# hassony2/homan

Hardware: AMD Instinct MI355X
Metric: optimisation iters/sec (30-frame 256^2 clip) (higher is better)
Workload: dtype f32

## Files before the change

### homan_amd/csrc/geometry.hip

```cpp
#include "hm_common.h"

__global__ __launch_bounds__(256) void k_rigid_fwd(const float* __restrict__ mesh, const float* __restrict__ rot6d,
                                                   const float* __restrict__ trans, const float* __restrict__ scale,
                                                   int abs_scale, int N, int V, float* __restrict__ rotmat,
                                                   float* __restrict__ verts, int clip_len)
{
    __shared__ float R[9];
    const int n = blockIdx.y;
    if (threadIdx.x == 0) {
        float r[9];
        rot6d_to_mat(rot6d + n * 6, r);
#pragma unroll
        for (int k = 0; k < 9; ++k) R[k] = r[k];
        if (blockIdx.x == 0 && rotmat)
#pragma unroll
            for (int k = 0; k < 9; ++k) rotmat[n * 9 + k] = r[k];
    }
    __syncthreads();
    const int v = blockIdx.x * blockDim.x + threadIdx.x;
    if (v >= V) return;
    float s = scale[n / clip_len];
    if (abs_scale) s = fabsf(s);
    const float* m = mesh + ((long)n * V + v) * 3;
    const float x = s * m[0], y = s * m[1], z = s * m[2];
    float* o = verts + ((long)n * V + v) * 3;
    const float* t = trans + n * 3;
    o[0] = x * R[0] + y * R[3] + z * R[6] + t[0];
    o[1] = x * R[1] + y * R[4] + z * R[7] + t[1];
    o[2] = x * R[2] + y * R[5] + z * R[8] + t[2];
}

struct SilGather {
    const double* parts;
    const int* adj_off;
    const int* adj_items;
    const float* cam_verts;
    const float* K;
    float orig_size;
    int F;
};
template <bool EXACT>
__global__ __launch_bounds__(1024) void k_rigid_bwd(const float* __restrict__ mesh, const float* __restrict__ rot6d,
                                                   const float* __restrict__ scale, int abs_scale, RigidTerms terms,
                                                   SilGather sil,
                                                   const float* __restrict__ g_rigid, const float* __restrict__ g_frame,
                                                   int frame_stride, float frame_scale, int N, int V,
                                                   float* __restrict__ g_mesh,
                                                   float* __restrict__ g_rot6d, float* __restrict__ g_trans,
                                                   float* __restrict__ g_scale_part, float* __restrict__ partials,
                                                   unsigned int* __restrict__ frame_cnt, int clip_len, double magic)
{
    HM_LATENCY_KERNEL();
    HM_STAMP_START(sil.parts ? 1 : 0);
    __shared__ float red13[16 * 13];
    __shared__ double red13d[EXACT ? 16 * 13 : 1];
    __shared__ int s_flag;
    const int n = blockIdx.x;
    float R[9];
    rot6d_to_mat(rot6d + n * 6, R);
    const float sraw = scale[n / clip_len];
    const float s = abs_scale ? fabsf(sraw) : sraw;
    float gfr[3] = {0.f, 0.f, 0.f};
    if (g_frame) {
#pragma unroll
        for (int c = 0; c < 3; ++c) gfr[c] = frame_scale * g_frame[(long)n * frame_stride + c];
    }
    float acc[13];
    double accd[13];
#pragma unroll
    for (int k = 0; k < 13; ++k) { acc[k] = 0.f; accd[k] = 0.0; }
    for (int v = blockIdx.y * blockDim.x + threadIdx.x; v < V; v += gridDim.y * blockDim.x) {
        const long o = ((long)n * V + v) * 3;
        const float m[3] = {mesh[o], mesh[o + 1], mesh[o + 2]};
        float gf[3] = {0.f, 0.f, 0.f}, gt[3];
#pragma unroll
        for (int k = 0; k < 5; ++k)
            if (terms.p[k]) {
                gf[0] += terms.w[k] * terms.p[k][o]; gf[1] += terms.w[k] * terms.p[k][o + 1]; gf[2] += terms.w[k] * terms.p[k][o + 2];
            }
        if (sil.parts) {
            double su = 0.0, sv = 0.0;
            const double2* pf = reinterpret_cast<const double2*>(sil.parts + (long)n * sil.F * 6);
            const int a1 = sil.adj_off[v + 1];
            for (int a = sil.adj_off[v]; a < a1; a += 8) {
                int item[8];
#pragma unroll
                for (int k = 0; k < 8; ++k) item[k] = a + k < a1 ? sil.adj_items[a + k] : -1;
                double2 g2[8];
#pragma unroll
                for (int k = 0; k < 8; ++k) g2[k] = item[k] >= 0 ? pf[item[k]] : make_double2(0.0, 0.0);
#pragma unroll
                for (int k = 0; k < 8; ++k) { su += g2[k].x; sv += g2[k].y; }
            }
            const float gu = (float)su, gv = (float)sv;
            const float* k = sil.K + n * 9;
            const float x = sil.cam_verts[o], y = sil.cam_verts[o + 1], z = sil.cam_verts[o + 2];
            const float zz = z + 1e-9f;
            const float du0 = gu * (2.0f / sil.orig_size), dv0 = -gv * (2.0f / sil.orig_size);
            const float dxn = k[0] * du0 + k[3] * dv0;
            const float dyn = k[1] * du0 + k[4] * dv0;
            gf[0] += dxn / zz;
            gf[1] += dyn / zz;
            gf[2] += -(dxn * x + dyn * y) / (zz * zz);
        }
        gt[0] = gf[0] + gfr[0]; gt[1] = gf[1] + gfr[1]; gt[2] = gf[2] + gfr[2];
        if (g_rigid) { gt[0] += g_rigid[o]; gt[1] += g_rigid[o + 1]; gt[2] += g_rigid[o + 2]; }
        const float dm[3] = {R[0] * gf[0] + R[1] * gf[1] + R[2] * gf[2], R[3] * gf[0] + R[4] * gf[1] + R[5] * gf[2],
                             R[6] * gf[0] + R[7] * gf[1] + R[8] * gf[2]};
        if (EXACT) {
#pragma unroll
            for (int i = 0; i < 3; ++i)
#pragma unroll
                for (int j = 0; j < 3; ++j) accd[3 * i + j] += hm_quant((s * m[i]) * gt[j], magic);
#pragma unroll
            for (int j = 0; j < 3; ++j) accd[9 + j] += hm_quant(gt[j], magic);
            accd[12] += hm_quant(m[0] * dm[0] + m[1] * dm[1] + m[2] * dm[2], magic);
        } else {
#pragma unroll
            for (int i = 0; i < 3; ++i)
#pragma unroll
                for (int j = 0; j < 3; ++j) acc[3 * i + j] += (s * m[i]) * gt[j];
#pragma unroll
            for (int j = 0; j < 3; ++j) acc[9 + j] += gt[j];
            acc[12] += m[0] * dm[0] + m[1] * dm[1] + m[2] * dm[2];
        }
        if (g_mesh) { g_mesh[o] = s * dm[0]; g_mesh[o + 1] = s * dm[1]; g_mesh[o + 2] = s * dm[2]; }
    }
    float tot[13];
    if (EXACT) {
        hm_block_sum_n_f64<13>(accd, red13d);
        if (gridDim.y > 1) {
            double* rec = reinterpret_cast<double*>(partials + ((long)n * gridDim.y + blockIdx.y) * 32);
            if (threadIdx.x == 0) {
#pragma unroll
                for (int k = 0; k < 13; ++k) __hip_atomic_store(rec + k, accd[k], __ATOMIC_RELAXED, __HIP_MEMORY_SCOPE_AGENT);
            }
            if (!hm_last_block(frame_cnt + n, gridDim.y, &s_flag)) return;
            if (threadIdx.x < 13 * gridDim.y)
                red13d[threadIdx.x] = __hip_atomic_load(reinterpret_cast<const double*>(partials + ((long)n * gridDim.y + threadIdx.x / 13) * 32) + threadIdx.x % 13,
                                                        __ATOMIC_RELAXED, __HIP_MEMORY_SCOPE_AGENT);
            __syncthreads();
            if (threadIdx.x == 0) {
#pragma unroll
                for (int k = 0; k < 13; ++k) accd[k] = 0.0;
                for (unsigned c = 0; c < gridDim.y; ++c)
#pragma unroll
                    for (int k = 0; k < 13; ++k) accd[k] += red13d[c * 13 + k];
            }
        }
#pragma unroll
        for (int k = 0; k < 13; ++k) tot[k] = (float)accd[k];
    } else {
#pragma unroll
    for (int k = 0; k < 13; ++k) tot[k] = acc[k];
    hm_block_sum_n<13>(tot, red13);
    if (gridDim.y > 1) {
        float* rec = partials + ((long)n * gridDim.y + blockIdx.y) * 32;
        if (threadIdx.x == 0) {
#pragma unroll
            for (int k = 0; k < 13; ++k) hm_partial_store(rec + k, tot[k]);
        }
        if (!hm_last_block(frame_cnt + n, gridDim.y, &s_flag)) return;
        if (threadIdx.x < 13 * gridDim.y)
            red13[threadIdx.x] = hm_partial_load(partials + ((long)n * gridDim.y + threadIdx.x / 13) * 32 + threadIdx.x % 13);
        __syncthreads();
        if (threadIdx.x == 0) {
#pragma unroll
            for (int k = 0; k < 13; ++k) tot[k] = 0.f;
            for (unsigned c = 0; c < gridDim.y; ++c)
#pragma unroll
                for (int k = 0; k < 13; ++k) tot[k] += red13[c * 13 + k];
        }
    }
    }
    if (threadIdx.x == 0) {
        float dr6[6];
        rot6d_backward(rot6d + n * 6, tot, dr6);
#pragma unroll
        for (int k = 0; k < 6; ++k) g_rot6d[n * 6 + k] = dr6[k];
#pragma unroll
        for (int k = 0; k < 3; ++k) g_trans[n * 3 + k] = tot[9 + k];
        if (g_scale_part) g_scale_part[n] = (abs_scale && sraw < 0.f) ? -tot[12] : tot[12];
    }
    HM_STAMP_END(sil.parts ? 1 : 0);
}

struct SmoothIn { const float* verts; float w; };
template <int NV, int MAXT>
__global__ __launch_bounds__(MAXT) void k_rigid_bwd_x(const float* __restrict__ mesh, const float* __restrict__ rot6d,
                                                     const float* __restrict__ scale, int abs_scale, RigidTerms terms,
                                                     SilGather sil, SmoothIn sm, int N, int V, float* __restrict__ g_rot6d,
                                                     float* __restrict__ g_trans, float* __restrict__ g_scale_part,
                                                     float* __restrict__ partials, unsigned int* __restrict__ frame_cnt,
                                                     int clip_len, double magic)
{
    HM_LATENCY_KERNEL();
    HM_STAMP_START(1);
    __shared__ double red13d[16 * 13];
    __shared__ int s_flag;
    const int n = blockIdx.x;
    float R[9];
    rot6d_to_mat(rot6d + n * 6, R);
    const float sraw = scale[n / clip_len];
    const float s = abs_scale ? fabsf(sraw) : sraw;
    const int fl = n % clip_len;
    const long row = (long)V * 3;
    const long scnt = (long)(clip_len - 1) * row;
    const float inv_cnt = scnt > 0 ? 1.0f / (float)scnt : 0.f;
    int vv[NV];
    bool ok[NV];
    int a0[NV], a1[NV];
    float m[NV][3], cv[NV][3], tv[NV][5][3], nb[NV][2][3];
#pragma unroll
    for (int j = 0; j < NV; ++j) {
        vv[j] = ((int)blockIdx.y * NV + j) * (int)blockDim.x + (int)threadIdx.x;
        ok[j] = vv[j] < V;
        const int v = ok[j] ? vv[j] : 0;
        const long o = ((long)n * V + v) * 3;
        a0[j] = sil.parts ? sil.adj_off[v] : 0;
        a1[j] = sil.parts ? sil.adj_off[v + 1] : 0;
#pragma unroll
        for (int c = 0; c < 3; ++c) {
            m[j][c] = mesh[o + c];
            cv[j][c] = sil.parts ? sil.cam_verts[o + c] : 0.f;
        }
#pragma unroll
        for (int k = 0; k < 5; ++k)
#pragma unroll
            for (int c = 0; c < 3; ++c) tv[j][k][c] = terms.p[k] ? terms.p[k][o + c] : 0.f;
#pragma unroll
        for (int c = 0; c < 3; ++c) {
            nb[j][0][c] = (sm.verts && fl + 1 < clip_len) ? sm.verts[o + row + c] : 0.f;
            nb[j][1][c] = (sm.verts && fl >= 1) ? sm.verts[o - row + c] : 0.f;
        }
    }
    float sv[NV][3];
#pragma unroll
    for (int j = 0; j < NV; ++j)
#pragma unroll
        for (int c = 0; c < 3; ++c) sv[j][c] = sm.verts ? sm.verts[((long)n * V + (ok[j] ? vv[j] : 0)) * 3 + c] : 0.f;
    int item[NV][8];
#pragma unroll
    for (int j = 0; j < NV; ++j)
#pragma unroll
        for (int k = 0; k < 8; ++k) item[j][k] = (ok[j] && a0[j] + k < a1[j]) ? sil.adj_items[a0[j] + k] : -1;
    double su[NV], sw[NV];
    {
        const double2* pf = reinterpret_cast<const double2*>(sil.parts + (long)n * sil.F * 6);
        double2 g2[NV][8];
#pragma unroll
        for (int j = 0; j < NV; ++j)
#pragma unroll
            for (int k = 0; k < 8; ++k) g2[j][k] = item[j][k] >= 0 ? pf[item[j][k]] : make_double2(0.0, 0.0);
#pragma unroll
        for (int j = 0; j < NV; ++j) {
            su[j] = 0.0; sw[j] = 0.0;
#pragma unroll
            for (int k = 0; k < 8; ++k) { su[j] += g2[j][k].x; sw[j] += g2[j][k].y; }
            for (int a = a0[j] + 8; ok[j] && a < a1[j]; ++a) {
                const double2 g = pf[sil.adj_items[a]];
                su[j] += g.x; sw[j] += g.y;
            }
        }
    }
    double accd[13];
#pragma unroll
    for (int k = 0; k < 13; ++k) accd[k] = 0.0;
#pragma unroll
    for (int j = 0; j < NV; ++j) {
        if (!ok[j]) continue;
        float gf[3] = {0.f, 0.f, 0.f}, gt[3];
        if (sm.verts) {
#pragma unroll
            for (int c = 0; c < 3; ++c) {
                float g = 0.f;
                if (fl + 1 < clip_len) { const float d = nb[j][0][c] - sv[j][c]; g -= d; }
                if (fl >= 1) g += sv[j][c] - nb[j][1][c];
                gf[c] += sm.w * (2.0f * g * inv_cnt);
            }
        }
#pragma unroll
        for (int k = 0; k < 5; ++k)
            if (terms.p[k]) {
                gf[0] += terms.w[k] * tv[j][k][0]; gf[1] += terms.w[k] * tv[j][k][1]; gf[2] += terms.w[k] * tv[j][k][2];
            }
        if (sil.parts) {
            const float gu = (float)su[j], gv = (float)sw[j];
            const float* k = sil.K + n * 9;
            const float x = cv[j][0], y = cv[j][1], z = cv[j][2];
            const float zz = z + 1e-9f;
            const float du0 = gu * (2.0f / sil.orig_size), dv0 = -gv * (2.0f / sil.orig_size);
            const float dxn = k[0] * du0 + k[3] * dv0;
            const float dyn = k[1] * du0 + k[4] * dv0;
            gf[0] += dxn / zz;
            gf[1] += dyn / zz;
            gf[2] += -(dxn * x + dyn * y) / (zz * zz);
        }
        gt[0] = gf[0] + 0.f; gt[1] = gf[1] + 0.f; gt[2] = gf[2] + 0.f;
        const float dm[3] = {R[0] * gf[0] + R[1] * gf[1] + R[2] * gf[2], R[3] * gf[0] + R[4] * gf[1] + R[5] * gf[2],
                             R[6] * gf[0] + R[7] * gf[1] + R[8] * gf[2]};
#pragma unroll
        for (int i = 0; i < 3; ++i)
#pragma unroll
            for (int q = 0; q < 3; ++q) accd[3 * i + q] += hm_quant((s * m[j][i]) * gt[q], magic);
#pragma unroll
        for (int q = 0; q < 3; ++q) accd[9 + q] += hm_quant(gt[q], magic);
        accd[12] += hm_quant(m[j][0] * dm[0] + m[j][1] * dm[1] + m[j][2] * dm[2], magic);
    }
    hm_block_sum_n_f64<13>(accd, red13d);
    if (gridDim.y > 1) {
        double* rec = reinterpret_cast<double*>(partials + ((long)n * gridDim.y + blockIdx.y) * 32);
        if (threadIdx.x == 0) {
#pragma unroll
            for (int k = 0; k < 13; ++k) __hip_atomic_store(rec + k, accd[k], __ATOMIC_RELAXED, __HIP_MEMORY_SCOPE_AGENT);
        }
        if (!hm_last_block(frame_cnt + n, gridDim.y, &s_flag)) return;
        if (threadIdx.x < 13 * gridDim.y)
            red13d[threadIdx.x] = __hip_atomic_load(reinterpret_cast<const double*>(partials + ((long)n * gridDim.y + threadIdx.x / 13) * 32) + threadIdx.x % 13,
                                                    __ATOMIC_RELAXED, __HIP_MEMORY_SCOPE_AGENT);
        __syncthreads();
        if (threadIdx.x == 0) {
#pragma unroll
            for (int k = 0; k < 13; ++k) accd[k] = 0.0;
            for (unsigned c = 0; c < gridDim.y; ++c)
#pragma unroll
                for (int k = 0; k < 13; ++k) accd[k] += red13d[c * 13 + k];
        }
    }
    if (threadIdx.x == 0) {
        float tot[13], dr6[6];
#pragma unroll
        for (int k = 0; k < 13; ++k) tot[k] = (float)accd[k];
        rot6d_backward(rot6d + n * 6, tot, dr6);
#pragma unroll
        for (int k = 0; k < 6; ++k) g_rot6d[n * 6 + k] = dr6[k];
#pragma unroll
        for (int k = 0; k < 3; ++k) g_trans[n * 3 + k] = tot[9 + k];
        if (g_scale_part) g_scale_part[n] = (abs_scale && sraw < 0.f) ? -tot[12] : tot[12];
    }
    HM_STAMP_END(1);
}

__global__ void k_scale_by(const float* __restrict__ in, const float* __restrict__ s, long n, float* __restrict__ out)
{
    const long i = (long)blockIdx.x * blockDim.x + threadIdx.x;
    if (i < n) out[i] = s[0] * in[i];
}
__global__ void k_sum_small(const float* __restrict__ parts, int n, float w0, const float* __restrict__ extra, float w1,
                            float* __restrict__ out)
{
    __shared__ float red[16];
    const int c = blockIdx.x;
    float a = 0.f;
    for (int i = threadIdx.x; i < n; i += blockDim.x) a += parts[(long)c * n + i];
    a = hm_block_sum(a, red);
    if (threadIdx.x == 0) out[c] = w0 * a + (extra ? w1 * extra[c] : 0.f);
}

extern "C" {
int hm_sum_small_clips(const float* parts, int n, float w0, const float* extra, float w1, float* out, int nclips,
                       hipStream_t stream)
{
    HM_CHECK_ARG(parts && out && n > 0 && nclips > 0);
    hipLaunchKernelGGL(k_sum_small, dim3(nclips), dim3(64), 0, stream, parts, n, w0, extra, w1, out);
    return hm_launch_status();
}
int hm_rigid_fwd_clips(const float* mesh, const float* rot6d, const float* trans, const float* scale, int abs_scale, int N,
                       int V, float* rotmat, float* verts, int clip_len, hipStream_t stream)
{
    HM_CHECK_ARG(mesh && rot6d && trans && scale && verts && N > 0 && V > 0 && HM_CLIP_LEN_OK(N, clip_len));
    hipLaunchKernelGGL(k_rigid_fwd, dim3(hm_cdiv(V, 256), N), dim3(256), 0, stream, mesh, rot6d, trans, scale,
                       abs_scale, N, V, rotmat, verts, clip_len ? clip_len : N);
    return hm_launch_status();
}
int hm_rigid_fwd(const float* mesh, const float* rot6d, const float* trans, const float* scale, int abs_scale, int N,
                 int V, float* rotmat, float* verts, hipStream_t stream)
{
    return hm_rigid_fwd_clips(mesh, rot6d, trans, scale, abs_scale, N, V, rotmat, verts, 0, stream);
}
#define RIGID_MAX_CHUNKS 16
size_t hm_rigid_workspace_bytes(int N) { return (((size_t)N * 4 + 255) & ~(size_t)255) + (size_t)N * RIGID_MAX_CHUNKS * 32 * 4; }
static int rigid_bwd_launch(const float* mesh, const float* rot6d, const float* scale, int abs_scale,
                            const float* const* g_terms, const float* weights, int n_terms, SilGather sil,
                            const float* g_rigid, const float* g_frame, int frame_stride, float frame_scale, int N, int V,
                            float* g_mesh, float* g_rot6d, float* g_trans, float* g_scale_part, void* workspace,
                            int clip_len, int exact, int sum_log2q, SmoothIn smooth, hipStream_t stream)
{
    HM_CHECK_ARG(sum_log2q <= 0 && sum_log2q >= -60);
    HM_CHECK_ARG(mesh && rot6d && scale && g_rot6d && g_trans && N > 0 && V > 0 && HM_CLIP_LEN_OK(N, clip_len));
    HM_CHECK_ARG(n_terms >= 0 && n_terms <= 5 && (n_terms == 0 || (g_terms && weights)));
    HM_CHECK_ARG(!g_frame || frame_stride >= 3);
    HM_CHECK_ARG(HM_ALIGNED(workspace, 8));
    RigidTerms t;
    for (int k = 0; k < 5; ++k) { t.p[k] = k < n_terms ? g_terms[k] : nullptr; t.w[k] = k < n_terms ? weights[k] : 0.f; }
    const int threads = exact ? 256 : (V > 512 ? 1024 : 256);
    const int chunks = workspace ? min(RIGID_MAX_CHUNKS, hm_cdiv(V, exact ? threads : 4 * threads)) : 1;
    unsigned int* cnt = (unsigned int*)workspace;
    float* partials = workspace ? (float*)((char*)workspace + (((size_t)N * 4 + 255) & ~(size_t)255)) : nullptr;
    const bool small = V <= RIGID_MAX_CHUNKS * 256;
    const int nv = small ? 1 : 2;
    const int thr = small ? 256 : 768;
    if (exact && !g_rigid && !g_frame && !g_mesh && (workspace ? V <= RIGID_MAX_CHUNKS * thr * nv : V <= thr * nv)) {
        const int ch = hm_cdiv(V, thr * nv);
        const double magic = hm_sum_magic(sum_log2q);
        if (nv == 2)
            hipLaunchKernelGGL((k_rigid_bwd_x<2, 768>), dim3(N, ch), dim3(thr), 0, stream, mesh, rot6d, scale,
                               abs_scale, t, sil, smooth, N, V, g_rot6d, g_trans, g_scale_part, partials, cnt, clip_len ? clip_len : N, magic);
        else
            hipLaunchKernelGGL((k_rigid_bwd_x<1, 1024>), dim3(N, ch), dim3(thr), 0, stream, mesh, rot6d, scale,
                               abs_scale, t, sil, smooth, N, V, g_rot6d, g_trans, g_scale_part, partials, cnt, clip_len ? clip_len : N, magic);
        return hm_launch_status();
    }
    HM_CHECK_ARG(!smooth.verts);
    if (exact)
        hipLaunchKernelGGL(k_rigid_bwd<true>, dim3(N, chunks), dim3(threads), 0, stream, mesh, rot6d, scale,
                           abs_scale, t, sil, g_rigid, g_frame, frame_stride, frame_scale, N, V, g_mesh, g_rot6d, g_trans,
// ... 67 lines not shown
```

### homan_amd/csrc/raster_sweep.hip

```cpp
#include "raster_ws.h"
#include "raster_hooks.h"

__device__ __forceinline__ float sample_grad(const float* __restrict__ gimg, int S, int is, int xi, int yi)
{
    return 0.25f * gimg[(long)((is - 1 - yi) >> 1) * S + (xi >> 1)];
}

__device__ __forceinline__ void sweep_term(float diff, int d1, float d1_cross, float k0, float k1, bool use0, bool use1,
                                           float eps, double magic, double& acc0, double& acc1)
{
    const float t = (float)d1 - d1_cross;
    const bool live = diff > 0.0f;
    float dist0 = k0 * t, dist1 = k1 * t;
    dist0 += (0.0f < dist0) ? eps : -eps;
    dist1 += (0.0f < dist1) ? eps : -eps;
    const float g0 = diff / dist0, g1 = diff / dist1;
    acc0 -= hm_quant((live && use0) ? g0 : 0.0f, magic);
    acc1 -= hm_quant((live && use1) ? g1 : 0.0f, magic);
}
__device__ __forceinline__ float sweep_item_scale(float c, float two_over_is, bool pow2, int is)
{
    return pow2 ? (c * 2.0f) * two_over_is : (c * 2.0f) / (float)is;
}

__device__ __forceinline__ void raster_reorder(int* __restrict__ wo_dyn, int* __restrict__ wo_tmp,
                                               const unsigned int* __restrict__ wg_cost, unsigned int* __restrict__ dyn_flag, int n,
                                               unsigned* __restrict__ s_hist)
{
    __shared__ unsigned s_wsum[4];
    __shared__ unsigned s_zero;
    const int tid = threadIdx.x, lane = tid & 63, wv = tid >> 6;
    for (int i = tid; i < 1024; i += 256) s_hist[i] = 0u;
    if (tid == 0) s_zero = 0u;
    __syncthreads();
    for (int base = 0; base < n; base += 256 * 16) {
        unsigned cv[16];
#pragma unroll
        for (int k = 0; k < 16; ++k) { const int i = base + 256 * k + tid; cv[k] = i < n ? wg_cost[i] : 0u; }
#pragma unroll
        for (int k = 0; k < 16; ++k)
            if (base + 256 * k + tid < n && cv[k] != 0u) atomicAdd(&s_hist[1023 - min(cv[k] >> 2, 1023u)], 1u);
    }
    __syncthreads();
    unsigned c[4], tot = 0u;
#pragma unroll
    for (int k = 0; k < 4; ++k) { c[k] = s_hist[4 * tid + k]; tot += c[k]; }
    const unsigned incl = (unsigned)hm_wave_scan_incl((int)tot);
    if (lane == 63) s_wsum[wv] = incl;
    __syncthreads();
    unsigned base0 = incl - tot;
    for (int q = 0; q < wv; ++q) base0 += s_wsum[q];
    const unsigned n_busy = s_wsum[0] + s_wsum[1] + s_wsum[2] + s_wsum[3];
#pragma unroll
    for (int k = 0; k < 4; ++k) { s_hist[4 * tid + k] = base0; base0 += c[k]; }
    __syncthreads();
    for (int base = 0; base < n; base += 256 * 16) {
        unsigned cv[16];
        int ev[16];
#pragma unroll
        for (int k = 0; k < 16; ++k) {
            const int i = base + 256 * k + tid;
            cv[k] = i < n ? wg_cost[i] : 0u;
            ev[k] = i < n ? wo_dyn[i] : 0;
        }
#pragma unroll
        for (int k = 0; k < 16; ++k) {
            const bool in = base + 256 * k + tid < n, zero = in && cv[k] == 0u;
            const unsigned long long zb = __ballot(zero);
            unsigned zbase = 0u;
            if (lane == 0 && zb) zbase = atomicAdd(&s_zero, (unsigned)__popcll(zb));
            zbase = (unsigned)__builtin_amdgcn_readfirstlane((int)zbase);
            if (zero) wo_tmp[n_busy + zbase + (unsigned)__popcll(zb & ((1ull << lane) - 1ull))] = ev[k];
            else if (in) wo_tmp[atomicAdd(&s_hist[1023 - min(cv[k] >> 2, 1023u)], 1u)] = ev[k];
        }
    }
    __threadfence();
    __syncthreads();
    for (int base = 0; base < n; base += 256 * 16) {
        int ev[16];
#pragma unroll
        for (int k = 0; k < 16; ++k) { const int i = base + 256 * k + tid; ev[k] = i < n ? __builtin_nontemporal_load(wo_tmp + i) : 0; }
#pragma unroll
        for (int k = 0; k < 16; ++k) { const int i = base + 256 * k + tid; if (i < n) wo_dyn[i] = ev[k]; }
    }
    if (tid == 0) *dyn_flag = 1u;
}

#ifdef SWEEP_STATS
__device__ unsigned long long g_sweep_n[16];
#endif
#ifdef SWEEP_UNIT_PROFILE
__device__ int g_unit_prof[65536][4];
#endif
struct SweepGeo {
    int var, edge, axis, d0r, dir, a_in, a_out;
    float p00, p01, p10, p11, p20, p21, num, d1_cross;
    bool geo;
};
struct SweepLite { int var, axis, d0r, a_in, a_out; bool geo, pos; };
__device__ __forceinline__ SweepLite sweep_item_lite(const SweepFace& fc, const int2* __restrict__ famtab, int j, bool mine, int is)
{
    SweepLite q;
    int fam = 0;
#pragma unroll
    for (int stp = 8; stp > 0; stp >>= 1)
        if ((int)fc.cum[fam + stp - 1] <= j) fam += stp;
    const int fstart = fam ? (int)fc.cum[fam - 1] : 0;
    q.var = fam >= 6 ? 1 : 0;
    const int ci = fam - 6 * q.var;
    q.axis = ci & 1;
    const int edge = ci >> 1, v0 = q.var ? 2 - edge : edge;
    const float p00 = (q.axis ? fc.py : fc.px)[v0], p01 = (q.axis ? fc.px : fc.py)[v0];
    const int2 ft = famtab[fam];
    const float slope = __int_as_float(ft.x);
    const bool lt = (ft.y >> 16) & 1;
    const int dir = q.axis == 0 ? (lt ? -1 : 1) : (lt ? 1 : -1);
    q.d0r = mine ? (ft.y & 0xffff) + (j - fstart) : 0;
    const float d1_cross = slope * ((float)q.d0r - p00) + p01;
    bool geo = mine && d1_cross > -8.0f && d1_cross < (float)is + 8.0f;
    const int d1_in = geo ? ((dir > 0) ? (int)floorf(d1_cross) : (int)ceilf(d1_cross)) : 0;
    const int d1_out = d1_in + dir;
    geo = geo && !(d1_in < 0 || is <= d1_in || d1_out < 0 || is <= d1_out);
    q.a_in = geo ? d1_in : 0;
    q.a_out = geo ? d1_out : 0;
    q.geo = geo;
    q.pos = dir > 0;
    return q;
}
__device__ __forceinline__ SweepGeo sweep_item_geo(const SweepFace& fc, int j, bool mine, int is,
                                                   const int2* __restrict__ famtab = nullptr)
{
    SweepGeo q;
    int fam = 0;
#pragma unroll
    for (int stp = 8; stp > 0; stp >>= 1)
        if ((int)fc.cum[fam + stp - 1] <= j) fam += stp;
    const int fstart = fam ? (int)fc.cum[fam - 1] : 0;
    q.var = fam >= 6 ? 1 : 0;
    const int ci = fam - 6 * q.var;
    q.edge = ci >> 1;
    q.axis = ci & 1;
    int v0 = q.edge, v1 = q.edge == 2 ? 0 : q.edge + 1, v2 = q.edge == 0 ? 2 : q.edge - 1;
    if (q.var) { v0 = 2 - v0; v1 = 2 - v1; v2 = 2 - v2; }
    const float* pa = q.axis ? fc.py : fc.px;
    const float* pb = q.axis ? fc.px : fc.py;
    q.p00 = pa[v0]; q.p01 = pb[v0]; q.p10 = pa[v1]; q.p11 = pb[v1]; q.p20 = pa[v2]; q.p21 = pb[v2];
    if (q.axis == 0) q.dir = (q.p00 < q.p10) ? -1 : 1;
    else q.dir = (q.p00 < q.p10) ? 1 : -1;
    const int d0_from = (int)fmaxf(ceilf(fminf(q.p00, q.p10)), 0.0f);
    q.num = q.p10 - q.p00;
    const float slope = famtab ? __int_as_float(famtab[fam].x) : (q.p11 - q.p01) / q.num;
    q.d0r = mine ? d0_from + (j - fstart) : 0;
    q.d1_cross = slope * ((float)q.d0r - q.p00) + q.p01;
    bool geo = mine && q.d1_cross > -8.0f && q.d1_cross < (float)is + 8.0f;
// ... 292 lines not shown
                                                 __popcll(__ballot(act1)), __popcll(__ballot(nb0 > 0)), __popcll(__ballot(nb1 > 0)),
                                                 (unsigned long long)hm_wave_scan_incl(nb0 + nb1)};
                if (lane == 63) { for (int k = 0; k < 7; ++k) atomicAdd(&g_sweep_n[k], c[k]); atomicAdd(&g_sweep_n[7], 1ull); }
            }
#endif
            const int n = nb0 + nb1;
            const int incl = hm_wave_scan_incl(n);
            const int npairs = __builtin_amdgcn_readlane(incl, 63);
            if (npairs > 0) {
                __builtin_amdgcn_wave_barrier();
                s_start[wv][lane] = incl - n;
                SweepItem it;
                it.x = d1_cross;
                it.c0 = sweep_item_scale(c0, inv_is, pow2, is);
                it.c1 = sweep_item_scale(c1, inv_is, pow2, is);
                it.base0 = (int)(lid[0] * is) + lo[0];
                it.base1 = (int)(lid[1] * is) + lo[1];
                it.nb0 = nb0;
                it.fn = fn;
                {
                    const int m0 = var ? 2 - edge : edge, k1 = edge == 2 ? 0 : edge + 1, m1 = var ? 2 - k1 : k1;
                    const int comp = axis ? 0 : 1;
                    it.meta = el | ((2 * m0 + comp) << 4) | ((2 * m1 + comp) << 7) | (use0 ? 1 << 10 : 0) |
                              (use1 ? 1 << 11 : 0) | (nb0 << 12);
                }
                s_item[wv][lane].it = it;
                wave_sync();
                const int* st = s_start[wv];
                int cur = -1;
                double acc0 = 0.0, acc1 = 0.0;
                int carry = 0;
#pragma unroll 1
                for (int base = 0; base < npairs; base += 256) {
                    SWEEP_HOOK_PAIR_ROUND(eps, base);
#ifdef SWEEP_STATS
                    if (lane == 0) atomicAdd(&g_sweep_n[11], 1ull);
#endif
#ifdef SWEEP_UNIT_PROFILE
                    ++up_rounds;
#endif
                    int4* hd = reinterpret_cast<int4*>(s_head[wv]);
                    hd[lane] = make_int4(0, 0, 0, 0);
                    wave_sync();
                    const int ex = incl - n;
                    if (n > 0 && ex >= base && ex < base + 256) s_head[wv][ex - base] = lane + 1;
                    wave_sync();
                    const int4 h = hd[lane];
                    int m[4];
                    m[0] = h.x; m[1] = max(m[0], h.y); m[2] = max(m[1], h.z); m[3] = max(m[2], h.w);
                    int inc = m[3];
                    inc = max(inc, __builtin_amdgcn_update_dpp(0, inc, 0x111, 0xf, 0xf, false));
                    inc = max(inc, __builtin_amdgcn_update_dpp(0, inc, 0x112, 0xf, 0xf, false));
                    inc = max(inc, __builtin_amdgcn_update_dpp(0, inc, 0x114, 0xf, 0xf, false));
                    inc = max(inc, __builtin_amdgcn_update_dpp(0, inc, 0x118, 0xf, 0xf, false));
                    inc = max(inc, __builtin_amdgcn_update_dpp(0, inc, 0x142, 0xa, 0xf, false));
                    inc = max(inc, __builtin_amdgcn_update_dpp(0, inc, 0x143, 0xc, 0xf, false));
                    int before = __builtin_amdgcn_update_dpp(0, inc, 0x138, 0xf, 0xf, false);
                    before = max(before, carry);
                    carry = max(carry, __builtin_amdgcn_readlane(inc, 63));
                    SweepSrc sc[4];
                    int qi[4], qmeta[4];
                    bool ph1[4];
#pragma unroll
                    for (int k = 0; k < 4; ++k) {
                        const int p = min(base + 4 * lane + k, npairs - 1);
                        const int i = max(max(before, m[k]) - 1, 0);
                        const int r = max(p - st[i], 0);
                        const SweepItem& qq = s_item[wv][i].it;
                        qmeta[k] = qq.meta;
                        const int q_nb0 = qmeta[k] >> 12;
                        ph1[k] = r >= q_nb0;
                        qi[k] = i;
                        OFF at = (OFF)qq.base0 + r;
                        if (ph1[k]) at = (OFF)qq.base1 + (r - q_nb0);
                        sc[k] = *hm_at<W32>(srcs, at);
                    }
#if SWEEP_COMBINE_MIN <= 64
                    if (base > 0) {
                        const int key0 = base + 4 * lane < npairs ? (qmeta[0] & 0x3ff) : cur;
                        sweep_combine_rows(cur, acc0, acc1, cur >= 0 && key0 != cur, lane);
                    }
#endif
#pragma unroll
                    for (int k = 0; k < 4; ++k) {
                        {
                            const bool valid = base + 4 * lane + k < npairs;
                            const SweepItem& qq = s_item[wv][qi[k]].it;
                            const int meta = qmeta[k], key = valid ? (meta & 0x3ff) : cur;
                            if (key != cur) {
                                if (cur >= 0) {
#ifdef SWEEP_HOOK_FLUSH
                                    SWEEP_HOOK_FLUSH(eps, s_fg[wv], lane, cur, acc0, acc1);
#else
                                    double* f = s_fg[wv][cur & 15];
                                    unsafeAtomicAdd(f + ((cur >> 4) & 7), acc0);
                                    unsafeAtomicAdd(f + ((cur >> 7) & 7), acc1);
#endif
                                }
                                cur = key;
                                acc0 = 0.0;
                                acc1 = 0.0;
                            }
                            const bool take = valid && (!ph1[k] || sc[k].owner == qq.fn);
                            sweep_term(take ? (ph1[k] ? sc[k].g : -sc[k].g) : 0.0f, sc[k].d1, qq.x, qq.c0, qq.c1,
                                       (meta & (1 << 10)) != 0, (meta & (1 << 11)) != 0, eps, magic, acc0, acc1);
                        }
                    }
                }
#if SWEEP_COMBINE_MIN <= 64
                if (npairs >= SWEEP_COMBINE_PAIRS) sweep_combine_rows(cur, acc0, acc1, cur >= 0, lane);
#endif
                if (cur >= 0) {
                    double* f = s_fg[wv][cur & 15];
                    unsafeAtomicAdd(f + ((cur >> 4) & 7), acc0);
                    unsafeAtomicAdd(f + ((cur >> 7) & 7), acc1);
                }
            }
            wave_sync();
            }
            if (lane < nfp) {
                const SweepFace& ff = s_face[wv][lane].f;
                const int off = ff.off, nit = (int)ff.cum[11];
                const int u_lo = off >> SWEEP_USHIFT, u_hi = (off + nit - 1) >> SWEEP_USHIFT;
                double v[6];
#pragma unroll
                for (int k = 0; k < 6; ++k) v[k] = s_fg[wv][lane][k];
                double* out = parts + (long)ff.bf * 6;
                if (u_lo == u_hi) {
#pragma unroll
                    for (int k = 0; k < 6; ++k) out[k] = v[k];
                } else {
#pragma unroll
                    for (int k = 0; k < 6; ++k) unsafeAtomicAdd(out + k, v[k]);
                }
            }
            if (nfp < SWEEP_PASS_FACES) break;
        }
#ifdef SWEEP_UNIT_PROFILE
        if (lane == 0 && u < 65536) {
            g_unit_prof[u][0] = (int)(wall_clock64() - up_t0); g_unit_prof[u][1] = up_pass;
            g_unit_prof[u][2] = up_trips | (up_q << 8); g_unit_prof[u][3] = up_rounds;
        }
#endif
    }
    if (ts_on) hm_ts_store(ts_slots, (long)blockIdx.x * 4 + (threadIdx.x >> 6), 1, (unsigned long long)wall_clock64());
}

__global__ void k_bwd_gather(const double* __restrict__ parts, const int* __restrict__ adj_off,
                             const int* __restrict__ adj_items, const float* __restrict__ verts,
                             const float* __restrict__ K, int B, int V, int F, float orig_size,
                             float* __restrict__ grad_ndc, float* __restrict__ grad_verts)
{
    const long i = (long)blockIdx.x * blockDim.x + threadIdx.x;
    if (i >= (long)B * V) return;
    const int b = (int)(i / V), v = (int)(i % V);
    double su = 0.0, sv = 0.0;
    const double2* pf = reinterpret_cast<const double2*>(parts + (long)b * F * 6);
    const int a1 = adj_off[v + 1];
    for (int a = adj_off[v]; a < a1; a += 8) {
        int item[8];
#pragma unroll
        for (int k = 0; k < 8; ++k) item[k] = a + k < a1 ? adj_items[a + k] : -1;
        double2 g2[8];
#pragma unroll
        for (int k = 0; k < 8; ++k) g2[k] = item[k] >= 0 ? pf[item[k]] : make_double2(0.0, 0.0);
#pragma unroll
        for (int k = 0; k < 8; ++k) { su += g2[k].x; sv += g2[k].y; }
    }
    const float gu = (float)su, gv = (float)sv;
    if (grad_ndc) { grad_ndc[3 * i] = gu; grad_ndc[3 * i + 1] = gv; grad_ndc[3 * i + 2] = 0.f; }
    const float* k = K + b * 9;
    const float x = verts[3 * i], y = verts[3 * i + 1], z = verts[3 * i + 2];
    const float zz = z + 1e-9f;
    const float du0 = gu * (2.0f / orig_size), dv0 = -gv * (2.0f / orig_size);
    const float dxn = k[0] * du0 + k[3] * dv0;
    const float dyn = k[1] * du0 + k[4] * dv0;
    grad_verts[3 * i] = dxn / zz;
    grad_verts[3 * i + 1] = dyn / zz;
    grad_verts[3 * i + 2] = -(dxn * x + dyn * y) / (zz * zz);
}

void hm_launch_sweep(const SilWs& w, int B, int F, int S, float eps, int sum_log2q, hipStream_t stream)
{
    const RasterTune& tune = hm_raster_tune();
    const int nsort = tune.raster_reorder ? 1 : 0;
    const int blocks = max(8, (min(min(hm_cdiv((long)B * F, 2), tune.sweep_blocks), TS_SWEEP_WGS - 8) & ~7) - 8 * nsort);
    const bool w32 = hm_offsets_fit_32(B, S);
    hipLaunchKernelGGL(w32 ? k_bwd_sweep<true> : k_bwd_sweep<false>, dim3(nsort + blocks), dim3(256), 0, stream, w.sweep,
                       w.idx_map, w.srcs, w.lrec, B, F, S, eps, hm_sum_magic(sum_log2q), w.parts, w.lsum, w.alpha16, w.counter + 24,
                       w.ts + 2 * (ts_raster_units(B, S) + ts_lines_units(B, F, S)), nsort, w.wo_dyn, w.wo_tmp, w.wg_cost,
                       w.counter + 26, (int)ts_raster_units(B, S));
}
void hm_launch_bwd_gather(const SilWs& w, const int* adj_off, const int* adj_items, const float* verts, const float* K, int B,
                          int V, int F, float orig_size, float* grad_ndc, float* grad_verts, hipStream_t stream)
{
    hipLaunchKernelGGL(k_bwd_gather, dim3(hm_cdiv((long)B * V, 256)), dim3(256), 0, stream, w.parts, adj_off, adj_items, verts,
                       K, B, V, F, orig_size, grad_ndc, grad_verts);
}
#ifdef SWEEP_UNIT_PROFILE
extern "C" int hm_debug_unit_profile(int* out)
{
    (void)hipDeviceSynchronize();
    (void)hipMemcpyFromSymbol(out, HIP_SYMBOL(g_unit_prof), sizeof(int) * 65536 * 4);
    static int z[65536][4];
    (void)hipMemcpyToSymbol(HIP_SYMBOL(g_unit_prof), z, sizeof(z));
    return HM_OK;
}
#endif
#ifdef SWEEP_STATS
extern "C" int hm_debug_sweep_stats(unsigned long long* out)
{
    unsigned long long z[16] = {0, 0, 0, 0, 0, 0, 0, 0, 0, 0, 0, 0, 0, 0, 0, 0};
    (void)hipDeviceSynchronize();
    (void)hipMemcpyFromSymbol(out, HIP_SYMBOL(g_sweep_n), sizeof(z));
    (void)hipMemcpyToSymbol(HIP_SYMBOL(g_sweep_n), z, sizeof(z));
    return HM_OK;
}
#endif
```

Measured before the change: 6774.

## Spread high-degree vertex adjacency tails across the wavefront

Per-vertex gathers of face gradient parts now handle the first 8 adjacent faces per thread, then hand any remaining adjacency entries to a new wave-cooperative routine. That routine uses ballot and readlane to process groups of four owning lanes at once, with all 64 lanes loading in parallel before a wave reduction. The aim is to remove divergence and serial latency when a few vertices have long adjacency lists. Dead lanes must now stay in the loop so the wave-level collectives work, and reduction order changes for the f64 sums.

```diff
diff --git a/homan_amd/csrc/fan_gather.h b/homan_amd/csrc/fan_gather.h
--- /dev/null
+++ b/homan_amd/csrc/fan_gather.h
@@ -0,0 +1,44 @@
+#pragma once
+#include "hm_common.h"
+
+#define HM_FAN_GROUP 4
+
+__device__ __forceinline__ void hm_fan_tail(const int* __restrict__ adj_items, const double2* __restrict__ parts2, long frame_off,
+                                            int start, int end, double& su, double& sw)
+{
+    unsigned long long mask = __ballot(start < end);
+    if (mask == 0) return;
+    const int lane = (int)(threadIdx.x & 63);
+    const int blo = (int)(unsigned)(unsigned long long)frame_off, bhi = (int)(unsigned)((unsigned long long)frame_off >> 32);
+    while (mask) {
+        int owner[HM_FAN_GROUP], s[HM_FAN_GROUP], e[HM_FAN_GROUP];
+        const double2* p[HM_FAN_GROUP];
+#pragma unroll
+        for (int g = 0; g < HM_FAN_GROUP; ++g) {
+            owner[g] = mask ? __builtin_ctzll(mask) : -1;
+            const int o = owner[g] < 0 ? 0 : owner[g];
+            s[g] = owner[g] < 0 ? 0 : __builtin_amdgcn_readlane(start, o);
+            e[g] = owner[g] < 0 ? 0 : __builtin_amdgcn_readlane(end, o);
+            p[g] = parts2 + (long)(((unsigned long long)(unsigned)__builtin_amdgcn_readlane(bhi, o) << 32) |
+                                   (unsigned long long)(unsigned)__builtin_amdgcn_readlane(blo, o));
+            mask &= mask - 1;
+        }
+        int item[HM_FAN_GROUP];
+#pragma unroll
+        for (int g = 0; g < HM_FAN_GROUP; ++g) item[g] = s[g] + lane < e[g] ? adj_items[s[g] + lane] : -1;
+        double2 v[HM_FAN_GROUP];
+#pragma unroll
+        for (int g = 0; g < HM_FAN_GROUP; ++g) v[g] = item[g] >= 0 ? p[g][item[g]] : make_double2(0.0, 0.0);
+#pragma unroll
+        for (int g = 0; g < HM_FAN_GROUP; ++g) {
+            if (owner[g] < 0) break;
+            for (int b = s[g] + 64; b < e[g]; b += 64) {
+                const int it = b + lane < e[g] ? adj_items[b + lane] : -1;
+                const double2 w = it >= 0 ? p[g][it] : make_double2(0.0, 0.0);
+                v[g].x += w.x; v[g].y += w.y;
+            }
+            const double tx = hm_wave_sum_f64(v[g].x), ty = hm_wave_sum_f64(v[g].y);
+            if (lane == owner[g]) { su += tx; sw += ty; }
+        }
+    }
+}
diff --git a/homan_amd/csrc/geometry.hip b/homan_amd/csrc/geometry.hip
--- a/homan_amd/csrc/geometry.hip
+++ b/homan_amd/csrc/geometry.hip
@@ -1,4 +1,5 @@
 #include "hm_common.h"
+#include "fan_gather.h"
 
 __global__ __launch_bounds__(256) void k_rigid_fwd(const float* __restrict__ mesh, const float* __restrict__ rot6d,
                                                    const float* __restrict__ trans, const float* __restrict__ scale,
@@ -69,8 +70,10 @@
     double accd[13];
 #pragma unroll
     for (int k = 0; k < 13; ++k) { acc[k] = 0.f; accd[k] = 0.0; }
-    for (int v = blockIdx.y * blockDim.x + threadIdx.x; v < V; v += gridDim.y * blockDim.x) {
-        const long o = ((long)n * V + v) * 3;
+    for (int vb = blockIdx.y * blockDim.x; vb < V; vb += gridDim.y * blockDim.x) {
+        const int v = vb + (int)threadIdx.x;
+        const bool live = v < V;
+        const long o = ((long)n * V + (live ? v : 0)) * 3;
         const float m[3] = {mesh[o], mesh[o + 1], mesh[o + 2]};
         float gf[3] = {0.f, 0.f, 0.f}, gt[3];
 #pragma unroll
@@ -78,20 +81,22 @@
             if (terms.p[k]) {
                 gf[0] += terms.w[k] * terms.p[k][o]; gf[1] += terms.w[k] * terms.p[k][o + 1]; gf[2] += terms.w[k] * terms.p[k][o + 2];
             }
+        double su = 0.0, sv = 0.0;
         if (sil.parts) {
-            double su = 0.0, sv = 0.0;
             const double2* pf = reinterpret_cast<const double2*>(sil.parts + (long)n * sil.F * 6);
-            const int a1 = sil.adj_off[v + 1];
-            for (int a = sil.adj_off[v]; a < a1; a += 8) {
-                int item[8];
-#pragma unroll
-                for (int k = 0; k < 8; ++k) item[k] = a + k < a1 ? sil.adj_items[a + k] : -1;
-                double2 g2[8];
-#pragma unroll
-                for (int k = 0; k < 8; ++k) g2[k] = item[k] >= 0 ? pf[item[k]] : make_double2(0.0, 0.0);
-#pragma unroll
-                for (int k = 0; k < 8; ++k) { su += g2[k].x; sv += g2[k].y; }
-            }
+            const int a0 = live ? sil.adj_off[v] : 0, a1 = live ? sil.adj_off[v + 1] : 0;
+            int item[8];
+#pragma unroll
+            for (int k = 0; k < 8; ++k) item[k] = a0 + k < a1 ? sil.adj_items[a0 + k] : -1;
+            double2 g2[8];
+#pragma unroll
+            for (int k = 0; k < 8; ++k) g2[k] = item[k] >= 0 ? pf[item[k]] : make_double2(0.0, 0.0);
+#pragma unroll
+            for (int k = 0; k < 8; ++k) { su += g2[k].x; sv += g2[k].y; }
+            hm_fan_tail(sil.adj_items, reinterpret_cast<const double2*>(sil.parts), (long)n * sil.F * 3, a0 + 8, a1, su, sv);
+        }
+        if (!live) continue;
+        if (sil.parts) {
             const float gu = (float)su, gv = (float)sv;
             const float* k = sil.K + n * 9;
             const float x = sil.cam_verts[o], y = sil.cam_verts[o + 1], z = sil.cam_verts[o + 2];
@@ -257,11 +262,11 @@
             su[j] = 0.0; sw[j] = 0.0;
 #pragma unroll
             for (int k = 0; k < 8; ++k) { su[j] += g2[j][k].x; sw[j] += g2[j][k].y; }
-            for (int a = a0[j] + 8; ok[j] && a < a1[j]; ++a) {
-                const double2 g = pf[sil.adj_items[a]];
-                su[j] += g.x; sw[j] += g.y;
-            }
-        }
+        }
+#pragma unroll
+        for (int j = 0; j < NV; ++j)
+            hm_fan_tail(sil.adj_items, reinterpret_cast<const double2*>(sil.parts), (long)n * sil.F * 3, a0[j] + 8, ok[j] ? a1[j] : 0,
+                        su[j], sw[j]);
     }
     double accd[13];
 #pragma unroll
diff --git a/homan_amd/csrc/raster_sweep.hip b/homan_amd/csrc/raster_sweep.hip
--- a/homan_amd/csrc/raster_sweep.hip
+++ b/homan_amd/csrc/raster_sweep.hip
@@ -1,5 +1,6 @@
 #include "raster_ws.h"
 #include "raster_hooks.h"
+#include "fan_gather.h"
 
 __device__ __forceinline__ float sample_grad(const float* __restrict__ gimg, int S, int is, int xi, int yi)
 {
@@ -598,21 +599,23 @@
                              float* __restrict__ grad_ndc, float* __restrict__ grad_verts)
 {
     const long i = (long)blockIdx.x * blockDim.x + threadIdx.x;
-    if (i >= (long)B * V) return;
-    const int b = (int)(i / V), v = (int)(i % V);
+    const bool live = i < (long)B * V;
+    const int b = live ? (int)(i / V) : 0, v = live ? (int)(i % V) : 0;
     double su = 0.0, sv = 0.0;
     const double2* pf = reinterpret_cast<const double2*>(parts + (long)b * F * 6);
-    const int a1 = adj_off[v + 1];
-    for (int a = adj_off[v]; a < a1; a += 8) {
+    const int a0 = live ? adj_off[v] : 0, a1 = live ? adj_off[v + 1] : 0;
+    {
         int item[8];
 #pragma unroll
-        for (int k = 0; k < 8; ++k) item[k] = a + k < a1 ? adj_items[a + k] : -1;
+        for (int k = 0; k < 8; ++k) item[k] = a0 + k < a1 ? adj_items[a0 + k] : -1;
         double2 g2[8];
 #pragma unroll
         for (int k = 0; k < 8; ++k) g2[k] = item[k] >= 0 ? pf[item[k]] : make_double2(0.0, 0.0);
 #pragma unroll
         for (int k = 0; k < 8; ++k) { su += g2[k].x; sv += g2[k].y; }
     }
+    hm_fan_tail(adj_items, reinterpret_cast<const double2*>(parts), (long)b * F * 3, a0 + 8, a1, su, sv);
+    if (!live) return;
     const float gu = (float)su, gv = (float)sv;
     if (grad_ndc) { grad_ndc[3 * i] = gu; grad_ndc[3 * i + 1] = gv; grad_ndc[3 * i + 2] = 0.f; }
     const float* k = K + b * 9;
```

New measurement: 6772. Within noise of the previous version (-0.0%).
